# guisongchen/vo_slam_test

Hardware: AMD Instinct MI355X
Metric: tracked frames/sec + local-BA LM-iters/sec (synthetic 640x480; value = tracked frames/sec: ORB extraction, frame post-processing, two guided searches with the culling / isInFrame steps between them and two pose-only solves per frame, one vo_tracker C call per batch) (higher is better)
Workload: dtype u8; 1 GPU; tracked frame: ORB extract (640x480, 8-level pyramid, 1000 kpts) + undistort/depth/grid + searchByProjection vs last frame + solvePoseOnlySE3 + cullingOutliersBeforeLocalMap + isInFrame (refined pose) + searchByProjection vs local map + solvePoseOnlySE3; frames, depth and map resident in HBM; parallelism=frames sharded x1, no collective, batches_in_flight=2

## Files before the change

### vo_slam_test_amd/csrc/guided.hip

```cpp
#include "vo_common.h"

#include <algorithm>
#include <cmath>
#include <vector>

namespace {

using namespace vo;

constexpr int kGridCols = 64, kGridRows = 48;
constexpr int kCells = kGridCols * kGridRows;
constexpr int TH_HIGH = 100, TH_LOW = 50;
constexpr int HISTO_LENGTH = 30;
constexpr int kMaxFeat = 16384;

enum GuidedMode {
  kModeFrame = 0,
  kModeLocalMap = 1,
  kModeKeyFrame = 2,
  kModeFuse = 3,
  kModeArea = 4,
  kModeSim3 = 5
};

struct FramesDev {
  int cap;
  float *x, *y, *angle, *uright, *depth;
  int *octave;
  uint8_t *desc;
  int *n;
  int *cell_start;
  unsigned short *cell_items;
  uint4 *srec;
  uint4 *sdesc;
  float xmin, ymin, gw, gh;
};

struct CamDev {
  float fx, fy, cx, cy, bf;
  double k[5];
  int distorted;
};

__global__ __launch_bounds__(256) void k_frame_post(FramesDev F, CamDev C, const vo_keypoint *kps, const uint8_t *desc,
                                                    const int *counts, int kp_capacity, const void *depth, int depth_kind,
                                                    long long depth_frame_stride, int depth_pitch, float inv_depth_scale,
                                                    int img_w, int img_h, int slot0, int *err) {
  const int f = blockIdx.y, i = blockIdx.x * 256 + threadIdx.x;
  const int n = min(counts[f], min(kp_capacity, F.cap));
  if (i == 0) {
    F.n[slot0 + f] = n;
    if (counts[f] > n) atomicOr(err, 2);
  }
  if (i >= n) return;
  const vo_keypoint kp = kps[(long long)f * kp_capacity + i];
  float ux = kp.x, uy = kp.y;
// ... 123 lines not shown
  const int *nq;
  int nq_all, stride;
};

struct GuidedParams {
  int mode;
  float radius, bf, ratio, dist_threshold;
  int direction, check_rot, n_levels, max_dist;
  float sf[16];
  int retry_below;
};

constexpr float kNarrowRadius = 20.f;
constexpr int kSlot = 32;

struct GuidedOut {
  unsigned *pool;
  unsigned short *rank;
  unsigned *ovf;
  unsigned short *ovf_rank;
  uint2 *qrec;
  int *ovf_used;
  int ovf_stride;
  int *best_idx;
  int *assigned;
  const uint8_t *fmask;
  unsigned *pushes;
  int *n_matches;
  int *retry_nq;
  int *err;
};

__device__ __forceinline__ unsigned row_min_u32(unsigned x) {
  x = min(x, (unsigned)__builtin_amdgcn_update_dpp((int)x, (int)x, 0xB1, 0xf, 0xf, false));
  x = min(x, (unsigned)__builtin_amdgcn_update_dpp((int)x, (int)x, 0x4E, 0xf, 0xf, false));
  x = min(x, (unsigned)__builtin_amdgcn_update_dpp((int)x, (int)x, 0x141, 0xf, 0xf, false));
  x = min(x, (unsigned)__builtin_amdgcn_update_dpp((int)x, (int)x, 0x140, 0xf, 0xf, false));
  return x;
}
__device__ __forceinline__ unsigned wave_min_u32(unsigned x) {
  x = row_min_u32(x);
  return min(min((unsigned)__builtin_amdgcn_readlane((int)x, 0), (unsigned)__builtin_amdgcn_readlane((int)x, 16)),
             min((unsigned)__builtin_amdgcn_readlane((int)x, 32), (unsigned)__builtin_amdgcn_readlane((int)x, 48)));
}

template <int G>
__device__ __forceinline__ unsigned group_min_u32(unsigned x) {
  if (G == 16) return row_min_u32(x);
#pragma unroll
  for (int o = G / 2; o >= 1; o >>= 1) x = min(x, (unsigned)__shfl_xor((int)x, o, G));
  return x;
}

template <int G>
__global__ __launch_bounds__(256) void k_guided_cand(FramesDev F, Queries Q, GuidedParams P, GuidedOut O, int slot0) {
  constexpr int kMaxCol = 64, QPB = 256 / G;
  __shared__ int s_pre[QPB][kMaxCol], s_base[QPB][kMaxCol];
  const int lane = threadIdx.x & 63, l16 = threadIdx.x & (G - 1), grp = threadIdx.x / G, sub = lane / G;
  const int f = blockIdx.y, q = blockIdx.x * QPB + grp;
  const int nq = Q.nq ? Q.nq[f] : Q.nq_all;
  if (nq < 0) return;
  const bool live = q < nq;
  const long long qo = (long long)f * Q.stride + (live ? q : 0);
  const int s = slot0 + f;
  const bool claims = P.mode == kModeFrame || P.mode == kModeLocalMap || P.mode == kModeKeyFrame || P.mode == kModeSim3;
  const unsigned flags = live ? Q.flags[qo] : 0u;
  const bool valid = (flags & 1u) != 0;
  const float u = Q.u[qo], v = Q.v[qo];
  const int lv = min(max(Q.level[qo], 0), 15);
  const float aux = Q.aux ? Q.aux[qo] : 0.f;
  const float q_angle = (P.check_rot && Q.angle) ? Q.angle[qo] : 0.f;
  const uint4 *qd4 = reinterpret_cast<const uint4 *>(Q.desc + qo * 32);
  const uint4 qa = qd4[0], qb = qd4[1];
  float rs;
  int lmin, lmax;
  if (P.mode == kModeFrame) {
    rs = P.radius * P.sf[lv];
    if (P.direction == 1) lmin = lv, lmax = P.n_levels;
    else if (P.direction == 2) lmin = 0, lmax = lv;
    else lmin = lv - 1, lmax = lv + 1;
  } else if (P.mode == kModeLocalMap) {
    float r = (Q.viewcos ? Q.viewcos[qo] : 1.f) > 0.998 ? 2.5f : 4.0f;
    r *= P.radius;
    rs = r * P.sf[lv];
    lmin = lv - 1, lmax = lv;
  } else if (P.mode == kModeKeyFrame) {
    rs = P.radius * P.sf[lv];
    lmin = lv - 1, lmax = lv + 1;
  } else {
    rs = P.radius * P.sf[lv];
    lmin = -(1 << 30), lmax = 1 << 30;
  }
  const int x0 = max(0, (int)floorf((u - F.xmin - rs) * F.gw));
  const int x1 = min(kGridCols - 1, (int)floorf((u - F.xmin + rs) * F.gw));
  const int y0 = max(0, (int)floorf((v - F.ymin - rs) * F.gh));
  const int y1 = min(kGridRows - 1, (int)floorf((v - F.ymin + rs) * F.gh));
  const bool window = valid && !(x0 >= kGridCols || x1 < 0 || y0 >= kGridRows || y1 < 0 || x1 < x0 || y1 < y0);
  const int *start = F.cell_start + (long long)s * (kCells + 1);
  const long long fo = (long long)s * F.cap, mo = (long long)f * F.cap;
  const int ncol = window ? x1 - x0 + 1 : 0;
  int T = 0;
  for (int cb = 0; cb < kMaxCol; cb += G) {
    const int c = cb + l16;
    int cbeg = 0, ccnt = 0;
    if (c < ncol) {
      cbeg = start[(x0 + c) * kGridRows + y0];
      ccnt = start[(x0 + c) * kGridRows + y1 + 1] - cbeg;
    }
    int incl = ccnt;
#pragma unroll
    for (int o = 1; o < G; o <<= 1) {
      const int t = __shfl_up(incl, o, G);
// ... 77 lines not shown
    return;
  }

  unsigned *slot = O.pool + ((long long)f * Q.stride + (live ? q : 0)) * kSlot;
  unsigned short *rslot = O.rank ? O.rank + ((long long)f * Q.stride + (live ? q : 0)) * kSlot : nullptr;
  int written = 0, rawbase = 0;
  for (int base = 0; base < Tmax; base += G) {
    const Item it = eval(base + l16);
    const unsigned pm = (unsigned)(__builtin_amdgcn_ballot_w64(it.pass) >> (G * sub)) & kGroupMask;
    const unsigned rm = (unsigned)(__builtin_amdgcn_ballot_w64(it.inraw) >> (G * sub)) & kGroupMask;
    const unsigned below = (1u << l16) - 1u;
    if (it.pass) {
      const int p = written + __popc(pm & below);
      if (p < kSlot) {
        slot[p] = (unsigned)it.idx | ((unsigned)it.dist << 14) | ((unsigned)(it.oct & 15) << 23) | ((unsigned)it.bin << 27);
        if (rslot) rslot[p] = (unsigned short)min(rawbase + __popc(rm & below), 65535);
      }
    }
    written += __popc(pm);
    rawbase += __popc(rm);
  }
  int ovf_off = 0;
  if (__builtin_amdgcn_ballot_w64(written > kSlot) != 0ull) {
    if (written > kSlot) {
      if (l16 == 0) ovf_off = atomicAdd(&O.ovf_used[f], written - kSlot);
      ovf_off = __shfl(ovf_off, 0, G);
      if (ovf_off + written - kSlot > O.ovf_stride) {
        if (l16 == 0) atomicOr(O.err, 1);
        written = kSlot;
      }
    }
    unsigned *ov = O.ovf + (long long)f * O.ovf_stride + ovf_off - kSlot;
    unsigned short *orv = O.ovf_rank ? O.ovf_rank + (long long)f * O.ovf_stride + ovf_off - kSlot : nullptr;
    int w2 = 0, r2 = 0;
    for (int base = 0; base < Tmax; base += G) {
      const Item it = eval(base + l16);
      const unsigned pm = (unsigned)(__builtin_amdgcn_ballot_w64(it.pass) >> (G * sub)) & kGroupMask;
      const unsigned rm = (unsigned)(__builtin_amdgcn_ballot_w64(it.inraw) >> (G * sub)) & kGroupMask;
      const unsigned below = (1u << l16) - 1u;
      if (it.pass) {
        const int p = w2 + __popc(pm & below);
        if (p >= kSlot && p < written) {
          ov[p] = (unsigned)it.idx | ((unsigned)it.dist << 14) | ((unsigned)(it.oct & 15) << 23) | ((unsigned)it.bin << 27);
          if (orv) orv[p] = (unsigned short)min(r2 + __popc(rm & below), 65535);
        }
      }
      w2 += __popc(pm);
      r2 += __popc(rm);
    }
  }
  if (live && l16 == 0) O.qrec[qo] = make_uint2((unsigned)written | ((flags >> 1) & 1u) << 31, (unsigned)ovf_off);
}

__global__ __launch_bounds__(256) void k_features_in_area(FramesDev F, int slot, int nq, const float *qu, const float *qv,
                                                          const float *qr, const int *qlo, const int *qhi, int *out,
                                                          int max_out, int *count) {
  const int lane = threadIdx.x & 63, l16 = threadIdx.x & 15, sub = lane >> 4;
  const int q = blockIdx.x * 16 + (threadIdx.x >> 4);
  const bool live = q < nq;
  const int qq = live ? q : 0;
  const float u = qu[qq], v = qv[qq], rs = qr[qq];
  const int lmin = qlo ? qlo[qq] : -(1 << 30), lmax = qhi ? qhi[qq] : (1 << 30);
  const int x0 = max(0, (int)floorf((u - F.xmin - rs) * F.gw));
  const int x1 = min(kGridCols - 1, (int)floorf((u - F.xmin + rs) * F.gw));
  const int y0 = max(0, (int)floorf((v - F.ymin - rs) * F.gh));
  const int y1 = min(kGridRows - 1, (int)floorf((v - F.ymin + rs) * F.gh));
  const bool window = live && !(x0 >= kGridCols || x1 < 0 || y0 >= kGridRows || y1 < 0);
  const int *start = F.cell_start + (long long)slot * (kCells + 1);
  const long long fo = (long long)slot * F.cap;
  int written = 0;
  const int ncol = window ? x1 - x0 + 1 : 0;
  int ncmax = ncol;
#pragma unroll
  for (int o = 32; o >= 1; o >>= 1) ncmax = max(ncmax, __shfl_xor(ncmax, o));
  for (int c = 0; c < ncmax; c++) {
    int cbeg = 0, cend = 0;
    if (c < ncol && y1 >= y0) cbeg = start[(x0 + c) * kGridRows + y0], cend = start[(x0 + c) * kGridRows + y1 + 1];
    int len = cend - cbeg, lenmax = len;
#pragma unroll
    for (int o = 32; o >= 1; o >>= 1) lenmax = max(lenmax, __shfl_xor(lenmax, o));
    for (int base = 0; base < lenmax; base += 16) {
      const int t = base + l16;
      bool hit = false;
      int idx = 0;
      if (t < len) {
        const uint4 r = F.srec[fo + cbeg + t];
        const float fx = __uint_as_float(r.x), fy = __uint_as_float(r.y);
        const int oct = (int)(r.w & 0xffu);
        idx = (int)(r.w >> 8);
        hit = !(oct < lmin || oct > lmax) && fabsf(fx - u) < rs && fabsf(fy - v) < rs;
      }
      const unsigned m = (unsigned)(__builtin_amdgcn_ballot_w64(hit) >> (16 * sub)) & 0xffffu;
      if (hit) {
        const int p = written + __popc(m & ((1u << l16) - 1u));
        if (p < max_out) out[(long long)q * max_out + p] = idx;
      }
      written += __popc(m);
    }
  }
  if (live && l16 == 0) count[q] = written;
}

__device__ __forceinline__ void lds_handoff() {
  asm volatile("s_waitcnt lgkmcnt(0)" ::: "memory");
  __builtin_amdgcn_wave_barrier();
}

__global__ __launch_bounds__(64) void k_guided_replay(FramesDev F, Queries Q, GuidedParams P, GuidedOut O, int slot0,
                                                      int batched_lds) {
  extern __shared__ __attribute__((aligned(16))) uint8_t rp_lds[];
  __shared__ int hist[32];
  const int lane = threadIdx.x, row = lane >> 4, l16 = lane & 15, f = blockIdx.x, s = slot0 + f;
  const int nf = F.n[s];
  const int nq = Q.nq ? Q.nq[f] : Q.nq_all;
  if (nq < 0) return;
  uint8_t *blocked = rp_lds;
  const int capA = (F.cap + 15) & ~15;
  unsigned short *asg = reinterpret_cast<unsigned short *>(rp_lds + capA);
  int *assigned = O.assigned + (long long)f * F.cap;
  const bool sim3 = P.mode == kModeSim3;
  for (int i = lane; i < nf; i += 64) {
    blocked[i] = O.fmask ? O.fmask[(long long)f * F.cap + i] : 0;
    const int a = sim3 ? -1 : assigned[i];
    asg[i] = (unsigned short)(a + 1);
  }
  if (lane < 32) hist[lane] = 0;
  lds_handoff();
  const uint2 *qrec = O.qrec + (long long)f * Q.stride;
  const unsigned *pool = O.pool + (long long)f * Q.stride * kSlot;
  const unsigned short *rkp = O.rank ? O.rank + (long long)f * Q.stride * kSlot : nullptr;
  const unsigned *ovf = O.ovf + (long long)f * O.ovf_stride;
  const unsigned short *ovr = O.ovf_rank ? O.ovf_rank + (long long)f * O.ovf_stride : nullptr;
  unsigned *pushes = O.pushes + (long long)f * Q.stride;
  const bool rot_on = P.check_rot && (P.mode == kModeFrame || P.mode == kModeKeyFrame);
  const bool want2 = P.mode == kModeLocalMap;
  int cnt = 0, npush = 0;
  constexpr unsigned kNone = 0xffffffffu;
  if (batched_lds && !sim3 && O.ovf_used[f] == 0) {
    int *tmpb = reinterpret_cast<int *>(rp_lds + capA + 2 * (size_t)capA);
    int *tmpw = tmpb + capA;
    for (int i = lane; i < capA; i += 64) tmpb[i] = 64, tmpw[i] = 0;
    lds_handoff();
    constexpr int R = kSlot;
    auto fetch64 = [&](int gb, unsigned (&rc)[R], unsigned &cw) {
      const int q = min(gb + lane, max(nq - 1, 0));
      cw = gb + lane < nq ? qrec[q].x : 0u;
      const uint4 *p4 = reinterpret_cast<const uint4 *>(pool + (long long)q * kSlot);
#pragma unroll
      for (int k = 0; k < R / 4; k++) {
        const uint4 v = p4[k];
        rc[4 * k] = v.x, rc[4 * k + 1] = v.y, rc[4 * k + 2] = v.z, rc[4 * k + 3] = v.w;
      }
    };
    unsigned recN[R], cwN;
    fetch64(0, recN, cwN);
    for (int gb = 0; gb < nq; gb += 64) {
      unsigned rec[R];
#pragma unroll
      for (int k = 0; k < R; k++) rec[k] = recN[k];
      const unsigned cw = cwN;
      fetch64(gb + 64, recN, cwN);
      const int cn = (int)(cw & 0x7fffffffu), ob = (int)(cw >> 31);
      const int cmax = ~(int)wave_min_u32(~(unsigned)cn);
      const int blocks = (P.mode == kModeFrame || P.mode == kModeLocalMap) ? ob : 1;
      bool unresolved = cn > 0;
      while (__builtin_amdgcn_ballot_w64(unresolved) != 0ull) {
        unsigned d1 = kNone, d2 = kNone, r1 = 0, r2 = 0;
#pragma unroll
        for (int c4 = 0; c4 < R / 4; c4++) {
          if (4 * c4 >= cmax) break;
#pragma unroll
          for (int u = 0; u < 4; u++) {
            const int pos = 4 * c4 + u;
            const unsigned rcd = rec[pos];
            const int idx = min((int)(rcd & 0x3fffu), capA - 1);
            const bool valid = unresolved & (pos < cn) & (blocked[idx] == 0);
            const unsigned d = valid ? ((rcd >> 14) & 0x1ffu) : kNone;
            const bool lt1 = d < d1, lt2 = d < d2;
            d2 = lt1 ? d1 : (lt2 ? d : d2), r2 = lt1 ? r1 : (lt2 ? rcd : r2);
            d1 = lt1 ? d : d1, r1 = lt1 ? rcd : r1;
          }
        }
        const int best = (int)d1, bidx = (int)(r1 & 0x3fffu);
        bool accept = unresolved && d1 != kNone;
        if (accept) {
          if (P.mode == kModeFrame) accept = best <= TH_HIGH;
          else if (P.mode == kModeLocalMap) {
            accept = best <= TH_HIGH;
            if (accept && d2 != kNone) {
              const int lv1 = (int)((r1 >> 23) & 0xfu), lv2 = (int)((r2 >> 23) & 0xfu);
              if (lv1 == lv2 && (float)best > P.ratio * (float)(int)d2) accept = false;
            }
          } else if (P.mode == kModeKeyFrame) accept = (float)best <= P.dist_threshold;
          else accept = best <= TH_LOW;
        }
        const bool blocker = accept && blocks != 0;
        if (blocker) atomicMin(&tmpb[bidx], lane);
        lds_handoff();
        bool stale = false;
        if (unresolved && d1 != kNone) {
          stale = tmpb[bidx] < lane;
          if (want2 && d2 != kNone) stale |= tmpb[(int)(r2 & 0x3fffu)] < lane;
        }
        const unsigned long long sm = __builtin_amdgcn_ballot_w64(stale);
        const int first_stale = sm ? (int)__builtin_ctzll(sm) : 64;
        const bool fin = unresolved && lane < first_stale, claim = fin && accept;
        if (claim) atomicMax(&tmpw[bidx], lane + 1);
        lds_handoff();
        const unsigned long long cm = __builtin_amdgcn_ballot_w64(claim);
        if (claim) {
          if (tmpw[bidx] == lane + 1) {
            asg[bidx] = (unsigned short)(gb + lane + 1);
            blocked[bidx] = (uint8_t)blocks;
          }
          if (rot_on) {
            const int bin = (int)(r1 >> 27);
            const int below = (int)__builtin_amdgcn_mbcnt_hi((unsigned)(cm >> 32), __builtin_amdgcn_mbcnt_lo((unsigned)cm, 0u));
            pushes[npush + below] = (unsigned)bidx | ((unsigned)bin << 16);
            atomicAdd(&hist[bin], 1);
          }
        }
        const int ncl = (int)__popcll(cm);
        cnt += ncl;
        if (rot_on) npush += ncl;
        lds_handoff();
        if (blocker) tmpb[bidx] = 64;
        if (claim) tmpw[bidx] = 0;
        unresolved = unresolved && !fin;
        lds_handoff();
      }
    }
  } else {
  struct Group { unsigned cw, oo, rec0, rec1; unsigned short rk0, rk1; };
  auto fetch = [&](int g0) {
    Group g{0u, 0u, 0u, 0u, 0, 0};
    const int q = min(g0 + row, max(nq - 1, 0));
    const uint2 qr = qrec[q];
    const long long sb = (long long)q * kSlot;
    g.rec0 = pool[sb + l16], g.rec1 = pool[sb + 16 + l16];
    if (rkp) g.rk0 = rkp[sb + l16], g.rk1 = rkp[sb + 16 + l16];
    g.cw = g0 + row < nq ? qr.x : 0u, g.oo = qr.y;
    return g;
  };
  constexpr int D = 4;
  auto replay_group = [&](const Group &g, int g0) {
    const int cn = (int)(g.cw & 0x7fffffffu), ob = (int)(g.cw >> 31);
    const int cmax = ~(int)wave_min_u32(~(unsigned)cn);
    if (cmax == 0) return;
    const int nch = (cmax + 15) >> 4;
    unsigned pending;
    {
      const unsigned long long m = __builtin_amdgcn_ballot_w64(cn > 0);
      pending = (unsigned)((m & 1ull) | ((m >> 15) & 2ull) | ((m >> 30) & 4ull) | ((m >> 45) & 8ull));
    }
    while (pending != 0u) {
      const bool mine = (pending >> row) & 1u;
      unsigned k1 = kNone, k2 = kNone, r1 = 0, r2 = 0;
      for (int c = 0; c < nch; c++) {
        unsigned rec = c == 0 ? g.rec0 : g.rec1;
        unsigned short rk = c == 0 ? g.rk0 : g.rk1;
        const int pos = 16 * c + l16;
        if (c >= 2) {
          rec = pos < cn ? ovf[g.oo + pos - kSlot] : 0u;
          rk = (ovr && pos < cn) ? ovr[g.oo + pos - kSlot] : (unsigned short)0;
        }
        const int idx = rec & 0x3fffu;
        const bool skip = !mine || pos >= cn || (sim3 ? (rk < nf && blocked[rk]) : blocked[idx]);
        unsigned key = skip ? kNone : (((rec >> 14) & 0x1ffu) << 16) | (unsigned)pos;
        const unsigned m1 = row_min_u32(key);
        const unsigned rr1 = (unsigned)__shfl((int)rec, (lane & 48) | (int)(m1 & 15u));
        unsigned m2 = kNone, rr2 = 0;
        if (want2) {
          if (key == m1) key = kNone;
          m2 = row_min_u32(key);
          rr2 = (unsigned)__shfl((int)rec, (lane & 48) | (int)(m2 & 15u));
        }
        if (m1 < k1) {
          if (k1 < m2) k2 = k1, r2 = r1; else k2 = m2, r2 = rr2;
          k1 = m1, r1 = rr1;
        } else if (m1 < k2) {
          k2 = m1, r2 = rr1;
        }
      }
      const int best = (int)(k1 >> 16), bidx = (int)(r1 & 0x3fffu);
// ... 15 lines not shown
#pragma unroll
      for (int r = 0; r < 3; r++) {
        const int a_r = __builtin_amdgcn_readlane((int)(accept && mine), 16 * r);
        const int b_r = __builtin_amdgcn_readlane(bidx, 16 * r), bl_r = __builtin_amdgcn_readlane(blocks, 16 * r);
        if (!(a_r && bl_r)) continue;
        if (row > r && mine) {
          const unsigned key0 = sim3 ? g.rk0 : (g.rec0 & 0x3fffu), key1 = sim3 ? g.rk1 : (g.rec1 & 0x3fffu);
          if ((l16 < cn && key0 == (unsigned)b_r) || (16 + l16 < cn && key1 == (unsigned)b_r) || cn > 32) stale = true;
        }
      }
      const unsigned long long sm = __builtin_amdgcn_ballot_w64(stale);
      int first_stale = 4;
      if (sm & 0xffff000000000000ull) first_stale = 3;
      if (sm & 0x0000ffff00000000ull) first_stale = 2;
      if (sm & 0x00000000ffff0000ull) first_stale = 1;
#pragma unroll
      for (int r = 0; r < 4; r++) {
        if (r >= first_stale || !((pending >> r) & 1u)) continue;
        const int a_r = __builtin_amdgcn_readlane((int)accept, 16 * r);
        if (a_r) {
          const int b_r = __builtin_amdgcn_readlane(bidx, 16 * r), bl_r = __builtin_amdgcn_readlane(blocks, 16 * r);
          const int bin = (int)((unsigned)__builtin_amdgcn_readlane((int)r1, 16 * r) >> 27);
          if (lane == 0) {
            asg[b_r] = (unsigned short)(g0 + r + 1);
            blocked[b_r] = (uint8_t)bl_r;
            if (rot_on) {
              pushes[npush] = (unsigned)b_r | ((unsigned)bin << 16);
              hist[bin]++;
            }
          }
        }
        cnt += a_r ? 1 : 0;
        npush += (a_r && rot_on) ? 1 : 0;
        pending &= ~(1u << r);
      }
      lds_handoff();
    }
  };
  Group nxt[D];
#pragma unroll
  for (int d = 0; d < D; d++) nxt[d] = fetch(4 * d);
  for (int gb = 0; gb < nq; gb += 4 * D) {
    Group cur[D];
#pragma unroll
    for (int d = 0; d < D; d++) cur[d] = nxt[d];
#pragma unroll
    for (int d = 0; d < D; d++) nxt[d] = fetch(gb + 4 * D + 4 * d);
#pragma unroll
    for (int d = 0; d < D; d++)
      if (gb + 4 * d < nq) replay_group(cur[d], gb + 4 * d);
  }
  }
  lds_handoff();
  if (npush > 0) {
    int m1 = 0, m2 = 0, m3 = 0, i1 = -1, i2 = -1, i3 = -1;
    for (int i = 0; i < HISTO_LENGTH; i++) {
      const int sz = hist[i];
      if (sz > m1) m3 = m2, i3 = i2, m2 = m1, i2 = i1, m1 = sz, i1 = i;
      else if (sz > m2) m3 = m2, i3 = i2, m2 = sz, i2 = i;
      else if (sz > m3) m3 = sz, i3 = i;
    }
    if (m2 < 0.1f * (float)m1) i2 = i3 = -1;
    else if (m3 < 0.1f * (float)m1) i3 = -1;
    __threadfence_block();
    for (int base = 0; base < npush; base += 64) {
      bool drop = false;
      if (base + lane < npush) {
        const unsigned p = pushes[base + lane];
        const int bin = (int)(p >> 16);
        if (bin != i1 && bin != i2 && bin != i3) {
          drop = true;
          asg[p & 0xffffu] = 0;
        }
      }
      cnt -= __popcll(__builtin_amdgcn_ballot_w64(drop));
    }
    lds_handoff();
  }
  const bool retry = O.retry_nq && cnt < P.retry_below;
  for (int i = lane; i < nf; i += 64) assigned[i] = retry ? -1 : (int)asg[i] - 1;
  if (lane == 0) {
    O.n_matches[f] = cnt, O.ovf_used[f] = 0;
    if (O.retry_nq) O.retry_nq[f] = retry ? nq : -1;
  }
}

__global__ __launch_bounds__(256) void k_guided_count(Queries Q, const int *best_idx, int *n_matches) {
  __shared__ int tot;
  const int f = blockIdx.x;
  const int nq = Q.nq ? Q.nq[f] : Q.nq_all;
  if (nq < 0) return;
  if (threadIdx.x == 0) tot = 0;
  __syncthreads();
  int c = 0;
  for (int q = threadIdx.x; q < nq; q += 256) c += best_idx[(long long)f * Q.stride + q] >= 0;
  if (c) atomicAdd(&tot, c);
  __syncthreads();
  if (threadIdx.x == 0) n_matches[f] = tot;
}

}

namespace vo {
void track_scatter_launch(int n_frames, int cap, int stride, const int *fn, int slot0, const int *assigned,
                          const double *qpoints, const uint8_t *qflags, double *fpoint, uint8_t *fhas, uint8_t *fobserved,
                          hipStream_t st);
void track_gather_launch(int n_frames, int cap, const int *fn, int slot0, const float *X, const float *Y, const float *UR,
                         const int *OCT, const double *fpoint, const uint8_t *fhas, const float *sf, double *pts, double *obs,
                         double *isg, int *ranges, int *index, hipStream_t st);
void track_scatter_gather_launch(int n_frames, int cap, int stride, const int *fn, int slot0, const int *assigned,
                                 const double *qpoints, const uint8_t *qflags, double *fpoint, uint8_t *fhas, uint8_t *fobserved,
                                 const float *X, const float *Y, const float *UR, const int *OCT, const float *sf, double *pts,
                                 double *obs, double *isg, int *ranges, int *index, hipStream_t st);
}

struct vo_frames {
  int max_frames = 0, cap = 0;
  FramesDev D{};
  CamDev cam{};
  float width = 640.f, height = 480.f;
  vo::OwnedDevBuf b_x, b_y, b_angle, b_ur, b_depth, b_oct, b_desc, b_n, b_cs, b_ci, b_srec, b_sdesc;
  vo::OwnedDevBuf b_pool, b_rank, b_ovf, b_ovfr, b_qrec, b_used, b_best, b_asg, b_push, b_nm, b_err, b_sf;
  size_t pool_stride = 0, replay_lds_attr = 0;
  float sf_host[16] = {0};
};

namespace {

int frames_alloc(vo_frames *h) {
  const size_t N = (size_t)h->max_frames * h->cap;
  VO_CHECK(h->b_x.reserve(N * 4));
  VO_CHECK(h->b_y.reserve(N * 4));
  VO_CHECK(h->b_angle.reserve(N * 4));
  VO_CHECK(h->b_ur.reserve(N * 4));
  VO_CHECK(h->b_depth.reserve(N * 4));
  VO_CHECK(h->b_oct.reserve(N * 4));
  VO_CHECK(h->b_desc.reserve(N * 32));
// ... 19 lines not shown
  h->D.xmin = xmin, h->D.ymin = ymin;
  h->D.gw = (float)kGridCols / (xmax - xmin);
  h->D.gh = (float)kGridRows / (ymax - ymin);
}

struct GuidedCall {
  int mode;
  float radius, bf, ratio, dist_threshold;
  int direction, check_rot, n_levels, max_dist;
  const float *scale_factors;
  int n_scale;
  int retry_below = 0;
  int *retry_nq = nullptr;
};

int guided_launch(vo_frames *h, int slot0, int n_frames, const Queries &Q, const GuidedCall &c, const uint8_t *fmask,
                  int *assigned, int *best_idx, int *n_matches, size_t pool_per_frame, hipStream_t st) {
  GuidedParams P{};
  P.mode = c.mode, P.radius = c.radius, P.bf = c.bf, P.ratio = c.ratio, P.dist_threshold = c.dist_threshold;
  P.direction = c.direction, P.check_rot = c.check_rot, P.n_levels = c.n_levels, P.max_dist = c.max_dist;
  for (int i = 0; i < 16; i++) P.sf[i] = i < c.n_scale ? c.scale_factors[i] : (c.n_scale > 0 ? c.scale_factors[c.n_scale - 1] : 1.f);
  const bool claims = c.mode == kModeFrame || c.mode == kModeLocalMap || c.mode == kModeKeyFrame || c.mode == kModeSim3;
  GuidedOut O{};
  O.best_idx = best_idx, O.assigned = assigned, O.fmask = fmask, O.n_matches = n_matches;
  P.retry_below = c.retry_below, O.retry_nq = c.retry_nq;
  if (!h->b_err.p) {
    VO_CHECK(h->b_err.reserve(64));
    VO_HIP_CHECK(hipMemsetAsync(h->b_err.p, 0, 64, st));
  }
  O.err = h->b_err.as<int>();
  if (claims) {
    const size_t slots = (size_t)n_frames * Q.stride * kSlot;
    VO_CHECK(h->b_pool.reserve(slots * 4 + 64));
    VO_CHECK(h->b_ovf.reserve((size_t)n_frames * pool_per_frame * 4 + 64));
    if (c.mode == kModeSim3) {
      VO_CHECK(h->b_rank.reserve(slots * 2 + 64));
      VO_CHECK(h->b_ovfr.reserve((size_t)n_frames * pool_per_frame * 2 + 64));
    }
    VO_CHECK(h->b_qrec.reserve((size_t)n_frames * Q.stride * 8 + 64));
    {
      void *before = h->b_used.p;
      VO_CHECK(h->b_used.reserve((size_t)h->max_frames * 4 + 64));
      if (h->b_used.p != before) VO_HIP_CHECK(hipMemsetAsync(h->b_used.p, 0, (size_t)h->max_frames * 4 + 64, st));
    }
    VO_CHECK(h->b_push.reserve((size_t)n_frames * Q.stride * 4 + 64));
    O.pool = h->b_pool.as<unsigned>(), O.ovf = h->b_ovf.as<unsigned>();
    O.rank = c.mode == kModeSim3 ? h->b_rank.as<unsigned short>() : nullptr;
    O.ovf_rank = c.mode == kModeSim3 ? h->b_ovfr.as<unsigned short>() : nullptr;
    O.qrec = h->b_qrec.as<uint2>(), O.ovf_used = h->b_used.as<int>(), O.pushes = h->b_push.as<unsigned>();
    O.ovf_stride = (int)pool_per_frame;
  }
  const int nq_max = Q.nq_all;
  if (nq_max > 0) {
    if (c.radius <= kNarrowRadius)
      hipLaunchKernelGGL(k_guided_cand<8>, dim3((nq_max + 31) / 32, n_frames), dim3(256), 0, st, h->D, Q, P, O, slot0);
    else
      hipLaunchKernelGGL(k_guided_cand<16>, dim3((nq_max + 15) / 16, n_frames), dim3(256), 0, st, h->D, Q, P, O, slot0);
  }
  if (claims) {
    const size_t capA = (size_t)((h->cap + 15) & ~15);
    const int batched = capA * 11 <= 160 * 1024 - 256 ? 1 : 0;
    const size_t lds = capA * 3 + (batched ? capA * 8 : 0);
    if (lds > 64 * 1024 && lds > h->replay_lds_attr) {
      VO_HIP_CHECK(hipFuncSetAttribute((const void *)k_guided_replay, hipFuncAttributeMaxDynamicSharedMemorySize, (int)lds));
      h->replay_lds_attr = lds;
    }
    hipLaunchKernelGGL(k_guided_replay, dim3(n_frames), dim3(64), lds, st, h->D, Q, P, O, slot0, batched);
  } else {
    hipLaunchKernelGGL(k_guided_count, dim3(n_frames), dim3(256), 0, st, Q, best_idx, n_matches);
  }
  VO_HIP_CHECK(hipGetLastError());
  return VO_OK;
}

}

extern "C" {

int vo_frames_create(vo_frames **out, int max_frames, int max_features) {
  if (!out || max_frames < 1 || max_features < 1 || max_features > kMaxFeat) {
    vo::set_error("vo_frames_create: 1 <= max_features <= %d", kMaxFeat);
    return VO_ERR_INVALID;
  }
  VO_CHECK(vo::ensure_device());
  vo_frames *h = new vo_frames();
  h->max_frames = max_frames, h->cap = max_features;
  const int rc = frames_alloc(h);
  if (rc != VO_OK) {
    vo_frames_destroy(h);
    return rc;
  }
  frames_set_bounds(h, 0.f, 0.f, 640.f, 480.f);
  *out = h;
  return VO_OK;
}

void vo_frames_destroy(vo_frames *h) { delete h; }

int vo_frames_set_camera(vo_frames *h, const float intrinsics[5], const float dist_coef[5], float width, float height) {
  if (!h || !intrinsics || !(width > 0) || !(height > 0)) return VO_ERR_INVALID;
  h->cam.fx = intrinsics[0], h->cam.fy = intrinsics[1], h->cam.cx = intrinsics[2], h->cam.cy = intrinsics[3];
  h->cam.bf = intrinsics[4];
  for (int i = 0; i < 5; i++) h->cam.k[i] = dist_coef ? (double)dist_coef[i] : 0.0;
  h->cam.distorted = dist_coef && dist_coef[0] != 0.0f;
  h->width = width, h->height = height;
  frames_set_bounds(h, 0.f, 0.f, width, height);
  return VO_OK;
}

int vo_frames_capacity(const vo_frames *h, int *max_frames, int *max_features) {
  if (!h) return VO_ERR_INVALID;
  if (max_frames) *max_frames = h->max_frames;
  if (max_features) *max_features = h->cap;
  return VO_OK;
}
// ... 77 lines not shown
  if (!h || slot < 0 || slot >= h->max_frames || n_queries < 0 || max_out < 0 ||
      (n_queries > 0 && (!u || !v || !radius || !out_count || (max_out > 0 && !out_idx))))
    return VO_ERR_INVALID;
  if (n_queries == 0) return VO_OK;
  thread_local vo::ScratchBuf du, dv, dr, dlo, dhi, dout, dcnt;
  hipStream_t st = vo::thread_stream();
  const char *what = "vo_frames_features_in_area";
  VO_CHECK(vo::upload(du, u, (size_t)n_queries * 4, st, what));
  VO_CHECK(vo::upload(dv, v, (size_t)n_queries * 4, st, what));
  VO_CHECK(vo::upload(dr, radius, (size_t)n_queries * 4, st, what));
  if (min_level) VO_CHECK(vo::upload(dlo, min_level, (size_t)n_queries * 4, st, what));
  if (max_level) VO_CHECK(vo::upload(dhi, max_level, (size_t)n_queries * 4, st, what));
  VO_CHECK(dout.reserve(std::max<size_t>((size_t)n_queries * max_out * 4, 64)));
  VO_CHECK(dcnt.reserve((size_t)n_queries * 4));
  hipLaunchKernelGGL(k_features_in_area, dim3((n_queries + 15) / 16), dim3(256), 0, st, h->D, slot, n_queries, du.as<float>(),
                     dv.as<float>(), dr.as<float>(), min_level ? dlo.as<int>() : nullptr, max_level ? dhi.as<int>() : nullptr,
                     dout.as<int>(), max_out, dcnt.as<int>());
  VO_HIP_CHECK(hipGetLastError());
  if (max_out > 0) VO_CHECK(vo::copy_d2h(out_idx, dout.p, (size_t)n_queries * max_out * 4, st, what));
  VO_CHECK(vo::copy_d2h(out_count, dcnt.p, (size_t)n_queries * 4, st, what));
  return vo::stream_sync(st, what);
}

int vo_match_guided_dev(vo_frames *h, int slot0, int n_frames, const vo_guided_queries *q, const vo_guided_params *p,
                        const uint8_t *dev_feature_mask, int32_t *dev_assigned, int32_t *dev_best_idx,
                        int32_t *dev_n_matches, size_t pool_per_frame, void *hip_stream) {
  if (!h || !q || !p || slot0 < 0 || n_frames < 1 || slot0 + n_frames > h->max_frames || q->n_queries < 0 ||
      q->stride < q->n_queries || !dev_n_matches || p->mode < 0 || p->mode > 5 || !p->scale_factors || p->n_levels < 1 ||
      p->n_levels > 16) {
    vo::set_error("vo_match_guided_dev: invalid argument");
    return VO_ERR_INVALID;
  }
  const bool claims = p->mode == kModeFrame || p->mode == kModeLocalMap || p->mode == kModeKeyFrame || p->mode == kModeSim3;
  if ((claims && !dev_assigned) || (!claims && !dev_best_idx) || q->n_queries > 65534) {
    vo::set_error("vo_match_guided_dev: missing output array or more than 65534 queries per frame");
    return VO_ERR_INVALID;
  }
  Queries Q{};
  Q.flags = q->flags, Q.u = q->u, Q.v = q->v, Q.aux = q->aux, Q.level = q->level, Q.angle = q->angle;
  Q.viewcos = q->viewcos, Q.desc = q->desc, Q.nq = q->n_per_frame, Q.nq_all = q->n_queries, Q.stride = q->stride;
  GuidedCall c{p->mode, p->radius, p->bf, p->ratio, p->dist_threshold, p->direction, p->check_rot, p->n_levels,
               p->max_dist, p->scale_factors, p->n_levels};
  if (p->retry_n_per_frame) {
    if (p->mode != kModeFrame) {
      vo::set_error("vo_match_guided_dev: retry_n_per_frame is for mode 0 (trackWithMotion's retry)");
      return VO_ERR_INVALID;
    }
    c.retry_below = p->retry_below, c.retry_nq = p->retry_n_per_frame;
  }
  if (pool_per_frame == 0) pool_per_frame = (size_t)std::max(q->n_queries, 1) * 16;
  return guided_launch(h, slot0, n_frames, Q, c, dev_feature_mask, dev_assigned, dev_best_idx, dev_n_matches,
                       pool_per_frame, (hipStream_t)hip_stream);
}

int vo_track_scatter_dev(vo_frames *h, int slot0, int n_frames, const int32_t *dev_assigned, const double *dev_query_points,
                         const uint8_t *dev_query_flags, int stride, double *dev_feature_points, uint8_t *dev_feature_has,
                         uint8_t *dev_feature_observed, void *hip_stream) {
  if (!h || slot0 < 0 || n_frames < 1 || slot0 + n_frames > h->max_frames || !dev_assigned || !dev_query_points ||
      !dev_query_flags || stride < 1 || !dev_feature_points || !dev_feature_has)
    return VO_ERR_INVALID;
  vo::track_scatter_launch(n_frames, h->cap, stride, h->D.n, slot0, dev_assigned, dev_query_points, dev_query_flags,
                           dev_feature_points, dev_feature_has, dev_feature_observed, (hipStream_t)hip_stream);
  VO_HIP_CHECK(hipGetLastError());
  return VO_OK;
}

int vo_track_gather_dev(vo_frames *h, int slot0, int n_frames, const double *dev_feature_points,
                        const uint8_t *dev_feature_has, const float *scale_factors, int n_levels, double *dev_points,
                        double *dev_obs, double *dev_inv_sigma, int32_t *dev_ranges, int32_t *dev_index, void *hip_stream) {
  if (!h || slot0 < 0 || n_frames < 1 || slot0 + n_frames > h->max_frames || !dev_feature_points || !dev_feature_has ||
      !scale_factors || n_levels < 1 || n_levels > 16 || !dev_points || !dev_obs || !dev_inv_sigma || !dev_ranges)
    return VO_ERR_INVALID;
  hipStream_t st = (hipStream_t)hip_stream;
  if (!h->b_sf.p) VO_CHECK(h->b_sf.reserve(64));
  if (memcmp(h->sf_host, scale_factors, (size_t)n_levels * 4) != 0) {
    memcpy(h->sf_host, scale_factors, (size_t)n_levels * 4);
    VO_HIP_CHECK(hipMemcpyAsync(h->b_sf.p, h->sf_host, 64, hipMemcpyHostToDevice, st));
  }
  vo::track_gather_launch(n_frames, h->cap, h->D.n, slot0, h->D.x, h->D.y, h->D.uright, h->D.octave, dev_feature_points,
                          dev_feature_has, h->b_sf.as<float>(), dev_points, dev_obs, dev_inv_sigma, dev_ranges, dev_index, st);
  VO_HIP_CHECK(hipGetLastError());
  return VO_OK;
}

int vo_track_scatter_gather_dev(vo_frames *h, int slot0, int n_frames, const int32_t *dev_assigned, const double *dev_query_points,
                                const uint8_t *dev_query_flags, int stride, double *dev_feature_points, uint8_t *dev_feature_has,
                                uint8_t *dev_feature_observed, const float *scale_factors, int n_levels, double *dev_points,
                                double *dev_obs, double *dev_inv_sigma, int32_t *dev_ranges, int32_t *dev_index, void *hip_stream) {
  if (!h || slot0 < 0 || n_frames < 1 || slot0 + n_frames > h->max_frames || !dev_assigned || !dev_query_points ||
      !dev_query_flags || stride < 1 || !dev_feature_points || !dev_feature_has || !scale_factors || n_levels < 1 ||
      n_levels > 16 || !dev_points || !dev_obs || !dev_inv_sigma || !dev_ranges)
    return VO_ERR_INVALID;
  hipStream_t st = (hipStream_t)hip_stream;
  if (!h->b_sf.p) VO_CHECK(h->b_sf.reserve(64));
  if (memcmp(h->sf_host, scale_factors, (size_t)n_levels * 4) != 0) {
    memcpy(h->sf_host, scale_factors, (size_t)n_levels * 4);
    VO_HIP_CHECK(hipMemcpyAsync(h->b_sf.p, h->sf_host, 64, hipMemcpyHostToDevice, st));
  }
  vo::track_scatter_gather_launch(n_frames, h->cap, stride, h->D.n, slot0, dev_assigned, dev_query_points, dev_query_flags,
                                  dev_feature_points, dev_feature_has, dev_feature_observed, h->D.x, h->D.y, h->D.uright,
                                  h->D.octave, h->b_sf.as<float>(), dev_points, dev_obs, dev_inv_sigma, dev_ranges, dev_index, st);
  VO_HIP_CHECK(hipGetLastError());
  return VO_OK;
}

int vo_match_guided_status(vo_frames *h, void *hip_stream) {
// ... 241 lines not shown
```

Before: 343,700 frames/s.

## Compact live queries in replay, skip dead frames in candidate kernel, batch loads

```diff
diff --git a/vo_slam_test_amd/csrc/guided.hip b/vo_slam_test_amd/csrc/guided.hip
--- a/vo_slam_test_amd/csrc/guided.hip
+++ b/vo_slam_test_amd/csrc/guided.hip
@@ -2,6 +2,7 @@
 
 #include <algorithm>
 #include <cmath>
+#include <type_traits>
 #include <vector>
 
 namespace {
@@ -231,12 +232,13 @@
   return x;
 }
 
+constexpr int kCandMaxCol = 64;
 template <int G>
-__global__ __launch_bounds__(256) void k_guided_cand(FramesDev F, Queries Q, GuidedParams P, GuidedOut O, int slot0) {
-  constexpr int kMaxCol = 64, QPB = 256 / G;
-  __shared__ int s_pre[QPB][kMaxCol], s_base[QPB][kMaxCol];
+__device__ __forceinline__ void guided_cand_frame(const FramesDev &F, const Queries &Q, const GuidedParams &P, const GuidedOut &O,
+                                                  int slot0, int f, int (*s_pre)[kCandMaxCol], int (*s_base)[kCandMaxCol]) {
+  constexpr int kMaxCol = kCandMaxCol, QPB = 256 / G;
   const int lane = threadIdx.x & 63, l16 = threadIdx.x & (G - 1), grp = threadIdx.x / G, sub = lane / G;
-  const int f = blockIdx.y, q = blockIdx.x * QPB + grp;
+  const int q = blockIdx.x * QPB + grp;
   const int nq = Q.nq ? Q.nq[f] : Q.nq_all;
   if (nq < 0) return;
   const bool live = q < nq;
@@ -420,6 +422,32 @@
   if (live && l16 == 0) O.qrec[qo] = make_uint2((unsigned)written | ((flags >> 1) & 1u) << 31, (unsigned)ovf_off);
 }
 
+template <int G>
+__global__ __launch_bounds__(256) void k_guided_cand(FramesDev F, Queries Q, GuidedParams P, GuidedOut O, int slot0) {
+  __shared__ int s_pre[256 / G][kCandMaxCol], s_base[256 / G][kCandMaxCol];
+  guided_cand_frame<G>(F, Q, P, O, slot0, blockIdx.y, s_pre, s_base);
+}
+
+constexpr int kCandRows = 64;
+template <int G>
+__global__ __launch_bounds__(256) void k_guided_cand_rows(FramesDev F, Queries Q, GuidedParams P, GuidedOut O, int slot0,
+                                                          int n_frames) {
+  __shared__ int s_pre[256 / G][kCandMaxCol], s_base[256 / G][kCandMaxCol];
+  const int lane = threadIdx.x & 63, rows = gridDim.y;
+  for (int f0 = blockIdx.y; f0 < n_frames; f0 += 64 * rows) {
+    const int fl = f0 + lane * rows;
+    const int nql = fl < n_frames ? Q.nq[fl] : -1;
+    unsigned long long in = __builtin_amdgcn_ballot_w64(nql >= 0);
+    while (in != 0ull) {
+      const int b = (int)__builtin_ctzll(in);
+      in &= in - 1ull;
+      guided_cand_frame<G>(F, Q, P, O, slot0, f0 + b * rows, s_pre, s_base);
+      __builtin_amdgcn_fence(__ATOMIC_ACQ_REL, "wavefront");
+      __builtin_amdgcn_wave_barrier();
+    }
+  }
+}
+
 __global__ __launch_bounds__(256) void k_features_in_area(FramesDev F, int slot, int nq, const float *qu, const float *qv,
                                                           const float *qr, const int *qlo, const int *qhi, int *out,
                                                           int max_out, int *count) {
@@ -474,6 +502,49 @@
   __builtin_amdgcn_wave_barrier();
 }
 
+#ifdef VO_REPLAY_STAMPS
+enum { kStWait, kStPropose, kStHandoff, kStCommit, kStPrologue, kStEpilogue, kStSteps, kStRounds, kStChunks, kStRecords, kStFrames, kStN };
+__device__ unsigned long long g_replay_stamps[2][kStN];
+#define RP_NOW(var) asm volatile("s_memrealtime %0\n\ts_waitcnt lgkmcnt(0)" : "=s"(var)::"memory")
+#define RP_STAMP(slot)           \
+  do {                           \
+    unsigned long long n_;       \
+    RP_NOW(n_);                  \
+    st_[slot] += n_ - tp_;       \
+    tp_ = n_;                    \
+  } while (0)
+#define RP_STAMP_DEP(slot, dep)                \
+  do {                                         \
+    asm volatile("" : "+v"(dep)::"memory");    \
+    RP_STAMP(slot);                            \
+  } while (0)
+#define RP_COUNT(slot, n) st_[slot] += (unsigned long long)(n)
+#else
+#define RP_STAMP(slot) do {} while (0)
+#define RP_STAMP_DEP(slot, dep) do {} while (0)
+#define RP_COUNT(slot, n) do {} while (0)
+#endif
+
+template <bool MASK>
+__device__ __forceinline__ void replay_load_state(const uint8_t *fm, const int *assigned, int nf, int lane, uint8_t *blocked,
+                                                  unsigned short *asg) {
+  for (int i0 = 0; i0 < nf; i0 += 64 * 8) {
+    int a[8];
+    unsigned b[8];
+#pragma unroll
+    for (int u = 0; u < 8; u++) {
+      const int i = min(i0 + 64 * u + lane, nf - 1);
+      a[u] = assigned[i];
+      b[u] = MASK ? (unsigned)fm[i] : 0u;
+    }
+#pragma unroll
+    for (int u = 0; u < 8; u++) {
+      const int i = i0 + 64 * u + lane;
+      if (i < nf) blocked[i] = (uint8_t)b[u], asg[i] = (unsigned short)(a[u] + 1);
+    }
+  }
+}
+
 __global__ __launch_bounds__(64) void k_guided_replay(FramesDev F, Queries Q, GuidedParams P, GuidedOut O, int slot0,
                                                       int batched_lds) {
   extern __shared__ __attribute__((aligned(16))) uint8_t rp_lds[];
@@ -482,15 +553,22 @@
   const int nf = F.n[s];
   const int nq = Q.nq ? Q.nq[f] : Q.nq_all;
   if (nq < 0) return;
+#ifdef VO_REPLAY_STAMPS
+  unsigned long long st_[kStN] = {0}, tp_;
+  RP_NOW(tp_);
+#endif
   uint8_t *blocked = rp_lds;
   const int capA = (F.cap + 15) & ~15;
   unsigned short *asg = reinterpret_cast<unsigned short *>(rp_lds + capA);
   int *assigned = O.assigned + (long long)f * F.cap;
   const bool sim3 = P.mode == kModeSim3;
-  for (int i = lane; i < nf; i += 64) {
-    blocked[i] = O.fmask ? O.fmask[(long long)f * F.cap + i] : 0;
-    const int a = sim3 ? -1 : assigned[i];
-    asg[i] = (unsigned short)(a + 1);
+  const uint8_t *fm = O.fmask ? O.fmask + (long long)f * F.cap : nullptr;
+  if (sim3) {
+    for (int i = lane; i < nf; i += 64) blocked[i] = fm ? fm[i] : 0, asg[i] = 0;
+  } else if (fm) {
+    replay_load_state<true>(fm, assigned, nf, lane, blocked, asg);
+  } else {
+    replay_load_state<false>(fm, assigned, nf, lane, blocked, asg);
   }
   if (lane < 32) hist[lane] = 0;
   lds_handoff();
@@ -509,10 +587,27 @@
     int *tmpw = tmpb + capA;
     for (int i = lane; i < capA; i += 64) tmpb[i] = 64, tmpw[i] = 0;
     lds_handoff();
+    unsigned short *qlist = reinterpret_cast<unsigned short *>(tmpw + capA);
+    int nlive = 0;
+    for (int g0 = 0; g0 < nq; g0 += 64 * 8) {
+      unsigned cw8[8];
+#pragma unroll
+      for (int u = 0; u < 8; u++) cw8[u] = qrec[min(g0 + 64 * u + lane, nq - 1)].x;
+#pragma unroll
+      for (int u = 0; u < 8; u++) {
+        const int q = g0 + 64 * u + lane;
+        const bool has = q < nq && (cw8[u] & 0x7fffffffu) != 0u;
+        const unsigned long long hm = __builtin_amdgcn_ballot_w64(has);
+        if (has) qlist[nlive + (int)__builtin_amdgcn_mbcnt_hi((unsigned)(hm >> 32), __builtin_amdgcn_mbcnt_lo((unsigned)hm, 0u))] = (unsigned short)q;
+        nlive += (int)__popcll(hm);
+      }
+    }
+    lds_handoff();
     constexpr int R = kSlot;
-    auto fetch64 = [&](int gb, unsigned (&rc)[R], unsigned &cw) {
-      const int q = min(gb + lane, max(nq - 1, 0));
-      cw = gb + lane < nq ? qrec[q].x : 0u;
+    auto fetch64 = [&](int gb, unsigned (&rc)[R], unsigned &cw, int &qn) {
+      const int q = qlist[min(gb + lane, max(nlive - 1, 0))];
+      qn = q;
+      cw = gb + lane < nlive ? qrec[q].x : 0u;
       const uint4 *p4 = reinterpret_cast<const uint4 *>(pool + (long long)q * kSlot);
 #pragma unroll
       for (int k = 0; k < R / 4; k++) {
@@ -521,18 +616,30 @@
       }
     };
     unsigned recN[R], cwN;
-    fetch64(0, recN, cwN);
-    for (int gb = 0; gb < nq; gb += 64) {
+    int qN = 0;
+    if (nlive > 0) fetch64(0, recN, cwN, qN);
+    RP_STAMP(kStPrologue);
+    for (int gb = 0; gb < nlive; gb += 64) {
+#ifdef VO_REPLAY_STAMPS
+      asm volatile("s_waitcnt vmcnt(0)" ::: "memory");
+      RP_STAMP(kStWait);
+#endif
       unsigned rec[R];
 #pragma unroll
       for (int k = 0; k < R; k++) rec[k] = recN[k];
       const unsigned cw = cwN;
-      fetch64(gb + 64, recN, cwN);
+      const int qcur = qN;
+      fetch64(gb + 64, recN, cwN, qN);
       const int cn = (int)(cw & 0x7fffffffu), ob = (int)(cw >> 31);
       const int cmax = ~(int)wave_min_u32(~(unsigned)cn);
       const int blocks = (P.mode == kModeFrame || P.mode == kModeLocalMap) ? ob : 1;
       bool unresolved = cn > 0;
+      RP_COUNT(kStSteps, 1);
+      RP_COUNT(kStChunks, (cmax + 3) >> 2);
+      RP_COUNT(kStRecords, __popcll(__builtin_amdgcn_ballot_w64(cn > 0)));
+      RP_STAMP(kStHandoff);
       while (__builtin_amdgcn_ballot_w64(unresolved) != 0ull) {
+        RP_COUNT(kStRounds, 1);
         unsigned d1 = kNone, d2 = kNone, r1 = 0, r2 = 0;
 #pragma unroll
         for (int c4 = 0; c4 < R / 4; c4++) {
@@ -562,6 +669,7 @@
           } else if (P.mode == kModeKeyFrame) accept = (float)best <= P.dist_threshold;
           else accept = best <= TH_LOW;
         }
+        RP_STAMP_DEP(kStPropose, d1);
         const bool blocker = accept && blocks != 0;
         if (blocker) atomicMin(&tmpb[bidx], lane);
         lds_handoff();
@@ -576,9 +684,10 @@
         if (claim) atomicMax(&tmpw[bidx], lane + 1);
         lds_handoff();
         const unsigned long long cm = __builtin_amdgcn_ballot_w64(claim);
+        RP_STAMP(kStHandoff);
         if (claim) {
           if (tmpw[bidx] == lane + 1) {
-            asg[bidx] = (unsigned short)(gb + lane + 1);
+            asg[bidx] = (unsigned short)(qcur + 1);
             blocked[bidx] = (uint8_t)blocks;
           }
           if (rot_on) {
@@ -592,12 +701,15 @@
         cnt += ncl;
         if (rot_on) npush += ncl;
         lds_handoff();
+        RP_STAMP(kStCommit);
         if (blocker) tmpb[bidx] = 64;
         if (claim) tmpw[bidx] = 0;
         unresolved = unresolved && !fin;
         lds_handoff();
+        RP_STAMP(kStHandoff);
       }
     }
+    RP_COUNT(kStFrames, 1);
   } else {
   struct Group { unsigned cw, oo, rec0, rec1; unsigned short rk0, rk1; };
   auto fetch = [&](int g0) {
@@ -719,6 +831,7 @@
   }
   }
   lds_handoff();
+  RP_STAMP(kStHandoff);
   if (npush > 0) {
     int m1 = 0, m2 = 0, m3 = 0, i1 = -1, i2 = -1, i3 = -1;
     for (int i = 0; i < HISTO_LENGTH; i++) {
@@ -730,17 +843,22 @@
     if (m2 < 0.1f * (float)m1) i2 = i3 = -1;
     else if (m3 < 0.1f * (float)m1) i3 = -1;
     __threadfence_block();
-    for (int base = 0; base < npush; base += 64) {
-      bool drop = false;
-      if (base + lane < npush) {
-        const unsigned p = pushes[base + lane];
-        const int bin = (int)(p >> 16);
-        if (bin != i1 && bin != i2 && bin != i3) {
-          drop = true;
-          asg[p & 0xffffu] = 0;
+    for (int base = 0; base < npush; base += 64 * 8) {
+      unsigned p8[8];
+#pragma unroll
+      for (int u = 0; u < 8; u++) p8[u] = pushes[min(base + 64 * u + lane, npush - 1)];
+#pragma unroll
+      for (int u = 0; u < 8; u++) {
+        bool drop = false;
+        if (base + 64 * u + lane < npush) {
+          const int bin = (int)(p8[u] >> 16);
+          if (bin != i1 && bin != i2 && bin != i3) {
+            drop = true;
+            asg[p8[u] & 0xffffu] = 0;
+          }
         }
+        cnt -= __popcll(__builtin_amdgcn_ballot_w64(drop));
       }
-      cnt -= __popcll(__builtin_amdgcn_ballot_w64(drop));
     }
     lds_handoff();
   }
@@ -750,6 +868,12 @@
     O.n_matches[f] = cnt, O.ovf_used[f] = 0;
     if (O.retry_nq) O.retry_nq[f] = retry ? nq : -1;
   }
+#ifdef VO_REPLAY_STAMPS
+  asm volatile("s_waitcnt vmcnt(0)" ::: "memory");
+  RP_STAMP(kStEpilogue);
+  if (lane == 0 && st_[kStFrames] && (P.mode == kModeFrame || P.mode == kModeLocalMap))
+    for (int i = 0; i < kStN; i++) atomicAdd(&g_replay_stamps[P.mode == kModeLocalMap][i], st_[i]);
+#endif
 }
 
 __global__ __launch_bounds__(256) void k_guided_count(Queries Q, const int *best_idx, int *n_matches) {
@@ -875,15 +999,21 @@
   }
   const int nq_max = Q.nq_all;
   if (nq_max > 0) {
-    if (c.radius <= kNarrowRadius)
-      hipLaunchKernelGGL(k_guided_cand<8>, dim3((nq_max + 31) / 32, n_frames), dim3(256), 0, st, h->D, Q, P, O, slot0);
-    else
-      hipLaunchKernelGGL(k_guided_cand<16>, dim3((nq_max + 15) / 16, n_frames), dim3(256), 0, st, h->D, Q, P, O, slot0);
+    const bool narrow = c.radius <= kNarrowRadius;
+    const dim3 grid(narrow ? (nq_max + 31) / 32 : (nq_max + 15) / 16, Q.nq ? std::min(n_frames, kCandRows) : n_frames);
+    if (Q.nq) {
+      if (narrow) hipLaunchKernelGGL(k_guided_cand_rows<8>, grid, dim3(256), 0, st, h->D, Q, P, O, slot0, n_frames);
+      else hipLaunchKernelGGL(k_guided_cand_rows<16>, grid, dim3(256), 0, st, h->D, Q, P, O, slot0, n_frames);
+    } else {
+      if (narrow) hipLaunchKernelGGL(k_guided_cand<8>, grid, dim3(256), 0, st, h->D, Q, P, O, slot0);
+      else hipLaunchKernelGGL(k_guided_cand<16>, grid, dim3(256), 0, st, h->D, Q, P, O, slot0);
+    }
   }
   if (claims) {
     const size_t capA = (size_t)((h->cap + 15) & ~15);
-    const int batched = capA * 11 <= 160 * 1024 - 256 ? 1 : 0;
-    const size_t lds = capA * 3 + (batched ? capA * 8 : 0);
+    const size_t qlist = ((size_t)std::max(Q.stride, 0) + 63) / 64 * 64 * 2;
+    const int batched = capA * 11 + qlist <= 160 * 1024 - 256 ? 1 : 0;
+    const size_t lds = capA * 3 + (batched ? capA * 8 + qlist : 0);
     if (lds > 64 * 1024 && lds > h->replay_lds_attr) {
       VO_HIP_CHECK(hipFuncSetAttribute((const void *)k_guided_replay, hipFuncAttributeMaxDynamicSharedMemorySize, (int)lds));
       h->replay_lds_attr = lds;
@@ -1067,6 +1197,18 @@
   return guided_launch(h, slot0, n_frames, Q, c, dev_feature_mask, dev_assigned, dev_best_idx, dev_n_matches,
                        pool_per_frame, (hipStream_t)hip_stream);
 }
+
+#ifdef VO_REPLAY_STAMPS
+int vo_debug_replay_stamps(unsigned long long *out, int reset) {
+  VO_HIP_CHECK(hipDeviceSynchronize());
+  if (out) VO_HIP_CHECK(hipMemcpyFromSymbol(out, HIP_SYMBOL(g_replay_stamps), sizeof(unsigned long long) * 2 * kStN));
+  if (reset) {
+    const unsigned long long zero[2 * kStN] = {0};
+    VO_HIP_CHECK(hipMemcpyToSymbol(HIP_SYMBOL(g_replay_stamps), zero, sizeof(zero)));
+  }
+  return VO_OK;
+}
+#endif
 
 int vo_track_scatter_dev(vo_frames *h, int slot0, int n_frames, const int32_t *dev_assigned, const double *dev_query_points,
                          const uint8_t *dev_query_flags, int stride, double *dev_feature_points, uint8_t *dev_feature_has,
```

Result: no change. 341,200 frames/s (-0.7%).
